# arcoslab/vfclik

Hardware: AMD Instinct MI355X
Metric: 7-DOF IK cycles/sec (whole node), batch=65536; max |qdot-qdot_ref| (higher is better)
Workload: dtype f64; 1 GPU; C3: batch=65536/GPU x 7-DOF lwr, goal + 8 decay repellers, float32 I/O, flags=0x0; parallelism=arm batch sharded over 1 GPU(s), no collective

## Files before the change

vfclik_amd/csrc/vfik_abi.cpp:

```cpp
#include <hip/hip_runtime.h>

#include <algorithm>
#include <cmath>
#include <cstdarg>
#include <cstdio>
#include <cstdlib>
#include <cstring>
#include <string>
#include <limits>
#include <vector>

#include "../../include/vfik.h"
#include "vfik_kernel.h"

namespace {

thread_local std::string g_err;

int fail(int code, const char* fmt, ...) {
    char buf[512];
    va_list ap;
    va_start(ap, fmt);
    vsnprintf(buf, sizeof buf, fmt, ap);
    va_end(ap);
// ... 381 lines not shown
    if (const char* e = std::getenv("VFIK_UNIFORM_IMAGE")) h->uni_allowed = std::atoi(e) != 0;
    if (const char* e = std::getenv("VFIK_MIXED_ORDERS")) h->mixed_allowed = std::atoi(e) != 0;
    if (const char* e = std::getenv("VFIK_DH_PATTERN")) h->dhp_allowed = std::atoi(e) != 0;
    if (const char* e = std::getenv("VFIK_ZERO_COPY_MAX")) h->zero_copy_max = (size_t)std::max(0L, std::atol(e));
    auto bail = [&](const char* what) { if (g_err.empty()) fail(VFIK_E_HIP, "%s failed", what); vfik_destroy(h); return (vfik_handle*)nullptr; };
    if (hipSetDevice(device) != hipSuccess) return bail("hipSetDevice");
    if (hipStreamCreateWithFlags(&h->stream, hipStreamNonBlocking) != hipSuccess) return bail("hipStreamCreate");
    {
        int cus = 0;
        if (hipDeviceGetAttribute(&cus, hipDeviceAttributeMultiprocessorCount, device) == hipSuccess && cus > 0) h->n_simd = 4 * cus;
    }
    const size_t B = batch;
    h->Bpad = (batch + 63) / 64 * 64;
    const size_t quad_plane = (size_t)h->Bpad * 4 * h->esz;
    {
        const size_t sz_goal = (4 + 6) * quad_plane;
        const size_t sz_kc = VFIK_KCONST_SLOT(vfik::kconst_bytes(n_joints));
        const size_t sz_lv = (size_t)((n_joints + 4) / 4) * h->Bpad * 4 * sizeof(float);
        const size_t sz_sf = (std::max<size_t>(1, (size_t)max_slots) + 1) / 2 * 3 * quad_plane;
        const size_t sz_su = (std::max<size_t>(1, (size_t)max_slots) + 1) * quad_plane;
        const size_t sz_sl = std::max<size_t>(1, (size_t)max_slots) * 2 * quad_plane;
        const size_t sz_or = (std::max<size_t>(1, (size_t)max_slots) + 15) / 16 * (size_t)h->Bpad * 16;
        if (dev_alloc(h, &h->d_arena, sz_goal + sz_kc + sz_lv + sz_sf + sz_su + sz_sl + sz_or, true)) return bail("alloc state arena");
        char* a0 = static_cast<char*>(h->d_arena);
        h->d_goal = a0;
        h->d_funnel = a0 + 4 * quad_plane;
        h->d_kconst = a0 + sz_goal;
        h->d_lastvec = reinterpret_cast<float*>(a0 + sz_goal + sz_kc);
        h->d_slots_fast = a0 + sz_goal + sz_kc + sz_lv;
        h->d_slots_uni = a0 + sz_goal + sz_kc + sz_lv + sz_sf;
        h->d_slots = a0 + sz_goal + sz_kc + sz_lv + sz_sf + sz_su;
        h->d_orders = a0 + sz_goal + sz_kc + sz_lv + sz_sf + sz_su + sz_sl;
    }
    {
        std::vector<char> plane((size_t)h->Bpad * 4 * h->esz, 0);
        for (int b = 0; b < h->Bpad; ++b) {
            if (io_dtype == 32) put<float>(plane, (size_t)b * 4 + 3, -std::numeric_limits<double>::infinity());
            else put<double>(plane, (size_t)b * 4 + 3, -std::numeric_limits<double>::infinity());
        }
        for (int sidx = 0; sidx < std::max(1, max_slots) + 1; ++sidx)
            if (hipMemcpyAsync(static_cast<char*>(h->d_slots_uni) + (size_t)sidx * plane.size(), plane.data(), plane.size(), hipMemcpyHostToDevice, h->stream) != hipSuccess)
                return bail("init uniform image");
        if (hipStreamSynchronize(h->stream) != hipSuccess) return bail("init uniform image");
    }
    if (dev_alloc(h, (void**)&h->d_mixw, 16 * sizeof(double), true)) return bail("alloc mixw");
    h->slots_per_arm.assign(B, 0);
    h->fast_slots_per_arm.assign(B, 0);
    h->arm_has_funnel.assign(B, 0);
    h->arm_pair_state.assign(B, 0);
    h->arm_safe.assign(B, 0.0);
    h->arm_force.assign(B, 0.0);
    h->arm_order.assign(B, -1);
#ifdef VFIK_STAMPS
    if (dev_alloc(h, (void**)&h->d_stamps, ((B + 63) / 64) * 10 * sizeof(unsigned long long), true)) return bail("alloc stamps");
#endif
    if (vfik_reset_state(h) != VFIK_OK) return bail("reset_state");
    vfik_params p{};
    p.speed_scale = 1.0; p.lambda = 0.1; p.rot_slowdown = 0.3; p.null_gain = 0.5; p.lookahead = 0.3;
    p.jl_gain = 0.5; p.max_vel = 1.0; p.jp_kp = 1.5; p.jp_delta = 0.087;
    for (double& w : p.wy) w = 1.0;
    for (double& w : p.wq) w = 1.0;
    p.mix_w[0] = p.mix_w[1] = 1.0;
    h->params = p;
    {
        std::vector<double> all(B, p.speed_scale);
        if (vfik_set_speed_scale(h, 0, batch, all.data()) != VFIK_OK) return bail("speed scale");
        h->speed_set = true;
    }
    if (hipStreamSynchronize(h->stream) != hipSuccess) return bail("sync");
    return h;
}

void vfik_destroy(vfik_handle* h) {
    if (!h) return;
    (void)hipSetDevice(h->device);
    if (h->stream) (void)hipStreamSynchronize(h->stream);
    void* ptrs[] = {h->d_arena, h->d_tool, h->d_ext, h->d_mixw, h->d_stamps, h->d_mixw_arm, h->d_track, h->d_wts, h->d_rollq[0], h->d_rollq[1], h->d_objects, h->d_obs_pose, h->d_obs_v6,
                    h->d_qalign};
    for (void* p : ptrs) if (p) (void)hipFree(p);
    if (h->arena_dev) (void)hipFree(h->arena_dev);
    if (h->arena_host) (void)hipHostFree(h->arena_host);
    for (auto& sc : h->sc) if (sc.p) (void)hipFree(sc.p);
    for (auto& ps : h->pipe) {
        if (ps.ev_out) (void)hipEventSynchronize(ps.ev_out);
        for (auto& s : ps.sc) if (s.p) (void)hipFree(s.p);
        for (hipEvent_t e : {ps.ev_in, ps.ev_k, ps.ev_out}) if (e) (void)hipEventDestroy(e);
    }
    if (h->s_in) (void)hipStreamDestroy(h->s_in);
    if (h->s_out) (void)hipStreamDestroy(h->s_out);
    if (h->own_stream && h->stream) (void)hipStreamDestroy(h->stream);
    delete h;
}

int vfik_set_stream(vfik_handle* h, void* hip_stream) {
    if (check_handle(h)) return VFIK_E_ARG;
    if (quiesce(h) != VFIK_OK) return VFIK_E_HIP;
    HIP_TRY(hipSetDevice(h->device));
    HIP_TRY(hipStreamSynchronize(h->stream));
    if (h->own_stream && h->stream) HIP_TRY(hipStreamDestroy(h->stream));
    h->stream = static_cast<hipStream_t>(hip_stream);
    h->own_stream = false;
    return VFIK_OK;
}

int vfik_set_chain(vfik_handle* h, const vfik_chain* c) {
    if (check_handle(h)) return VFIK_E_ARG;
    if (quiesce(h) != VFIK_OK) return VFIK_E_HIP;
// ... 782 lines not shown
}

int vfik_dev_free(vfik_handle* h, void* p) {
    if (check_handle(h)) return VFIK_E_ARG;
    HIP_TRY(hipSetDevice(h->device));
    HIP_TRY(hipFree(p));
    return VFIK_OK;
}

int vfik_memcpy_h2d(vfik_handle* h, void* dst, const void* src, size_t bytes) {
    if (check_handle(h)) return VFIK_E_ARG;
    HIP_TRY(hipSetDevice(h->device));
    HIP_TRY(hipMemcpyAsync(dst, src, bytes, hipMemcpyHostToDevice, h->stream));
    HIP_TRY(hipStreamSynchronize(h->stream));
    return VFIK_OK;
}

int vfik_memcpy_d2h(vfik_handle* h, void* dst, const void* src, size_t bytes) {
    if (check_handle(h)) return VFIK_E_ARG;
    HIP_TRY(hipSetDevice(h->device));
    HIP_TRY(hipMemcpyAsync(dst, src, bytes, hipMemcpyDeviceToHost, h->stream));
    HIP_TRY(hipStreamSynchronize(h->stream));
    return VFIK_OK;
}

int vfik_time_steps(vfik_handle* h, const vfik_io* io, int warmup, int steps, float* ms_total) {
    if (check_handle(h)) return VFIK_E_ARG;
    if (!ms_total || steps < 1 || warmup < 0) return fail(VFIK_E_ARG, "vfik_time_steps: bad arguments");
    HIP_TRY(hipSetDevice(h->device));
    for (int i = 0; i < warmup; ++i) {
        int rc = vfik_step(h, io);
        if (rc != VFIK_OK) return rc;
    }
    hipEvent_t t0, t1;
    HIP_TRY(hipEventCreate(&t0));
    HIP_TRY(hipEventCreate(&t1));
    HIP_TRY(hipEventRecord(t0, h->stream));
    for (int i = 0; i < steps; ++i) {
        int rc = vfik_step(h, io);
        if (rc != VFIK_OK) { (void)hipEventDestroy(t0); (void)hipEventDestroy(t1); return rc; }
    }
    HIP_TRY(hipEventRecord(t1, h->stream));
    HIP_TRY(hipEventSynchronize(t1));
    HIP_TRY(hipEventElapsedTime(ms_total, t0, t1));
    (void)hipEventDestroy(t0);
    (void)hipEventDestroy(t1);
    return VFIK_OK;
}

#ifdef VFIK_STAMPS
int vfik_debug_read_stamps(vfik_handle* h, unsigned long long* dst) {
    if (check_handle(h)) return VFIK_E_ARG;
    HIP_TRY(hipStreamSynchronize(h->stream));
    HIP_TRY(hipMemcpy(dst, h->d_stamps, (size_t)((h->B + 63) / 64) * 10 * sizeof(unsigned long long), hipMemcpyDeviceToHost));
    return VFIK_OK;
}
#endif

int vfik_slots_in_use(vfik_handle* h) { return h ? h->slots_used : VFIK_E_ARG; }

int vfik_field_path(vfik_handle* h) {
    if (!h) return VFIK_E_ARG;
    if (h->fast_order < 0) return 0;
    return h->any_funnel ? 2 : 1;
}

long vfik_launch_epoch(vfik_handle* h) { return h ? h->epoch : (long)VFIK_E_ARG; }

int vfik_dh_pattern(vfik_handle* h) { return h ? ((h->plain && !h->tool_per_arm && !h->d_wts) ? h->dhp : 0) : VFIK_E_ARG; }

int vfik_mixed_orders(vfik_handle* h) {
    if (!h) return VFIK_E_ARG;
    return (h->fast_order >= 0 && h->mixed) ? 1 : 0;
}

int vfik_uniform_repellers(vfik_handle* h) {
    if (!h) return VFIK_E_ARG;
    return (h->fast_order >= 0 && h->uni_ok && h->uni_allowed) ? 1 : 0;
}

int vfik_set_small_batch_kernel(vfik_handle* h, int max_batch) {
    if (check_handle(h)) return VFIK_E_ARG;
    if (max_batch < 0) return fail(VFIK_E_ARG, "max_batch must be >= 0");
    ++h->epoch;
    h->sub8_max_batch = max_batch;
    h->sub8_max_batch_full = max_batch;
    h->sub8_max_batch_ns = max_batch;
    return VFIK_OK;
}

long vfik_small_batch_launches(vfik_handle* h) { return h ? h->sub8_launches : -1; }

int vfik_launched_kernels(vfik_handle* h, char* buf, int len) {
    if (check_handle(h)) return VFIK_E_ARG;
    if (h->launched_lost) return fail(VFIK_E_STATE, "more than %d distinct cycle kernels launched since the last vfik_launched_kernels", vfik_handle::LAUNCHED_MAX);
    std::string all;
    for (int i = 0; i < h->launched_n; ++i) {
        all += vfik::cycle_kernel_name(h->launched[i].p, h->n, h->io_dtype, h->launched[i].ns);
        all += '\n';
    }
    if (!buf) return (int)all.size();
    if (len < (int)all.size() + 1) return fail(VFIK_E_ARG, "vfik_launched_kernels: %d bytes needed", (int)all.size() + 1);
    std::memcpy(buf, all.c_str(), all.size() + 1);
    h->launched_n = 0;
    return (int)all.size();
}

// ... 4 lines not shown
```

vfclik_amd/csrc/vfik_kernel.h:

```cpp
#pragma once
#include <algorithm>
#include <cstddef>
#include <cstdio>
#include <string>

#include <hip/hip_runtime.h>
#include <stdint.h>

#include "../../include/vfik_types.h"

#ifndef VFIK_NJ_LIST
#define VFIK_NJ_LIST X(6) X(7) X(10) X(14)
#endif

namespace vfik {

template <int NJ>
struct KConst {
    double base[12];
    struct DH { double off, crev, cprs, sprs, qd, d, a, ca, sa, pad; } dh[NJ];
    double tail_c, tail_s, tail_e;
    double rep_safe;
    double speed, lambda2, rot_slow, null_gain, lookahead, max_vel;
    double cos_slow;
// ... 7 lines not shown
    double q_hi[NJ];
    double q_mid[NJ];
    double inv_half[NJ];
    double jl_k[NJ];
    unsigned prismatic_mask;
    unsigned pad0;
    static constexpr int KIN_BYTES = (12 + 10 * NJ + 4 + 10 + VFIK_MIX_CHANNELS + 12 + 6 + NJ) * 8;
    static constexpr int KIN_ROWS = (KIN_BYTES + 1023) / 1024;
};
#define VFIK_KCONST_REP_FORCE_OFF ((12 + 9) * 8)
#define VFIK_KCONST_REP_SAFE_OFF(nj) ((12 + 10 * (nj) + 3) * 8)
static_assert(offsetof(KConst<7>, rep_safe) == VFIK_KCONST_REP_SAFE_OFF(7) && offsetof(KConst<14>, rep_safe) == VFIK_KCONST_REP_SAFE_OFF(14), "KConst::rep_safe");
static_assert(offsetof(KConst<7>, dh) + offsetof(KConst<7>::DH, pad) == VFIK_KCONST_REP_FORCE_OFF, "KConst::dh[0].pad");
static_assert(offsetof(KConst<7>, wq) + 7 * 8 == KConst<7>::KIN_BYTES && offsetof(KConst<14>, wq) + 14 * 8 == KConst<14>::KIN_BYTES, "KConst::wq closes the LDS-copied block");
static_assert(KConst<7>::KIN_BYTES <= 1024 && KConst<6>::KIN_BYTES <= 1024 && KConst<10>::KIN_BYTES <= 2048 && KConst<14>::KIN_BYTES <= 2048, "the copied block keeps its row count");
template <int NJ> struct KTab { static constexpr int OFFSET = ((int)sizeof(KConst<NJ>) + 1023) / 1024 * 1024; };

template <int NJ, int DHP> struct DhPattern { static constexpr unsigned SWAP = 0, NONE = 0, D0 = 0, OFF0 = 0, OFFPI = 0; static constexpr bool BASE_I = false; };
template <> struct DhPattern<7, 1> { static constexpr unsigned SWAP = 0x3Fu, NONE = 0x40u, D0 = 0x2Au, OFF0 = 0x15u, OFFPI = 0x6Au; static constexpr bool BASE_I = true; };
template <> struct DhPattern<14, 1> {
    static constexpr unsigned SWAP = 0x1FBFu, NONE = 0x2040u, D0 = 0x152Au, OFF0 = 0xA95u, OFFPI = 0x356Au;
    static constexpr bool BASE_I = true;
};
template <> struct DhPattern<6, 1> { static constexpr unsigned SWAP = 0x1Du, NONE = 0x20u, D0 = 0x16u, OFF0 = 0x27u, OFFPI = 0x18u; static constexpr bool BASE_I = true; };
int dh_pattern_of(int nj, unsigned swap, unsigned none, unsigned d0, unsigned off0, unsigned offpi, bool base_identity);

template <typename T> struct Stage {
    static constexpr int PRE = sizeof(T) == 8 ? 4 : 8;
    static constexpr int Q16 = (int)sizeof(T) / 4;
    static constexpr int QBYTES = 4 * (int)sizeof(T);
    static constexpr int QSTEP = Q16 * 1024;
    static constexpr int QPCF = 3 * PRE / 2;
    static constexpr int GOAL_OFF = 0, SLOT_OFF = 4 * QSTEP, Q_OFF = (4 + QPCF) * QSTEP;
    __host__ __device__ static constexpr int qbytes(int nj) { return nj * (int)sizeof(T); }
    __host__ __device__ static constexpr int q16(int nj) { return qbytes(nj) / 16; }
    __host__ __device__ static constexpr int qrem(int nj) { return qbytes(nj) % 16; }
    __host__ __device__ static constexpr int qregion(int nj) { return q16(nj) * 1024 + qrem(nj) * 64; }
    __host__ __device__ static constexpr int kin_rows(int nj) { return ((12 + 10 * nj + 4 + 10 + VFIK_MIX_CHANNELS + 12 + 6 + nj) * 8 + 1023) / 1024; }
    __host__ __device__ static constexpr int kin_off(int nj) { return Q_OFF + qregion(nj); }
    __host__ __device__ static constexpr int tab_off(int nj) { return kin_off(nj) + kin_rows(nj) * 1024; }
    __host__ __device__ static constexpr int lean_bytes(int nj) { return tab_off(nj) + 1024; }
    __host__ __device__ static constexpr int slot_off(int idx, int nj) {
        return idx < QPCF ? SLOT_OFF + idx * QSTEP : lean_bytes(nj) + (idx - QPCF) * QSTEP;
    }
    __host__ __device__ static constexpr int tool_off(int nj) { return lean_bytes(nj) + (2 * PRE - QPCF) * QSTEP; }
    __host__ __device__ static constexpr int mixw_off(int nj) { return tool_off(nj) + 3 * QSTEP; }
    __host__ __device__ static constexpr int bytes(int nj) { return mixw_off(nj) + 2 * QSTEP; }
};

#define VFIK_ROLL_MAX_NJ 7
#ifndef VFIK_HEAVY_MIN_NJ
#define VFIK_HEAVY_MIN_NJ 12
#endif

struct KArgs {
    int B;
    int Bpad;
    int slots_used;
    int fast_order;
    unsigned flags;
    int tool_stride;
    int plain;
    int block;
    const void* q;
    const void* goal;
    const void* slots;
    const void* slots_fast;
    const void* tool;
    const void* null_control;
    const void* ext;
    const void* mixw;
    const double* wts;
    const void* q_ref;
    const void* q_cmded;
    float* lastvec;
    void* qdot_vf;
    void* qdot_null;
    void* qdot_out;
    void* pose;
    void* pose_nt;
    void* v6;
    void* qdist;
    void* goal_dist;
    int* status;
    unsigned long long* stamps;
    const void* kc;
    void* q_out;
    double dt;
    int n_cycles;
    int clamp;
    int status_or;
    const int* active;
    const void* q_lo;
    const void* q_hi;
    void* q_ref_out;
    int sub8_max_batch;
    int sub8_max_batch_ns;
    int sub8_max_batch_full;
    int n_simd;
    const void* funnel;
    int slots_used_fast;
    int has_funnel;
    const void* arena;
    int uni;
    int uni_planes;
    int waves2;
// ... 233 lines not shown
```

vfclik_amd/csrc/vfik_kernel.hip:

```cpp
#include "vfik_kernel.h"

#include <algorithm>
#include <cmath>
#include <cstring>
#include <type_traits>

namespace vfik {
#define VFIK_CAT2(a, b) a##b
#define VFIK_CAT(a, b) VFIK_CAT2(a, b)
#if defined(VFIK_ONLY_NJ) && VFIK_ONLY_NJ >= VFIK_HEAVY_MIN_NJ
void VFIK_CAT(launch_heavy_nj, VFIK_ONLY_NJ)(int io_dtype, bool ns, const KArgs& a, const CyclePlan& p, hipStream_t stream);
#endif
namespace {

constexpr double EPS_LEN = 1e-12;
constexpr double D_FLOOR = 1e-9;
constexpr double MAG_CAP = 1e6;

__device__ __forceinline__ double rcp_nr(double x) {
    double y = __builtin_amdgcn_rcp(x);
    double e = __builtin_fma(-x, y, 1.0);
    y = __builtin_fma(y, e, y);
    e = __builtin_fma(-x, y, 1.0);
    return __builtin_fma(y, e, y);
// ... 487 lines not shown
        double z[NJ];
        descent(z);
        double c[6];
#pragma unroll
        for (int r = 0; r < 6; ++r) c[r] = 0.0;
#pragma unroll
        for (int i = 0; i < NJ; ++i)
#pragma unroll
            for (int r = 0; r < 6; ++r) c[r] += Jm[i][r] * z[i];
#pragma unroll
        for (int r = 0; r < 6; ++r)
#pragma unroll
            for (int i = 0; i < NJ; ++i) z[i] -= c[r] * Jm[i][r];
#pragma unroll
        for (int i = 0; i < NJ; ++i) qn[i] += z[i];
    }
    return advanced;
}


template <typename T, int NJ>
__device__ __forceinline__ int q_lds_off(int b, int lane) {
    constexpr int n16 = Stage<T>::q16(NJ), rem = Stage<T>::qrem(NJ);
    if (b < n16 * 16) return (b >> 4) * 1024 + lane * 16 + (b & 15);
    const int rb = b - n16 * 16;
    (void)rem;
    return n16 * 1024 + (rb >> 2) * 256 + lane * 4 + (rb & 3);
}

typedef __attribute__((address_space(1))) const void* GPtr;
typedef __attribute__((address_space(3))) void* LPtr;

template <typename T>
__device__ __forceinline__ void stage_quad(const char* gbase, unsigned voff, char* region, int off) {
    const char* gsrc = gbase + (long)(int)voff;
    __builtin_amdgcn_global_load_lds((GPtr)gsrc, (LPtr)(region + off), 16, 0, 2);
    if (Stage<T>::Q16 == 2) __builtin_amdgcn_global_load_lds((GPtr)(gsrc + 16), (LPtr)(region + off + 1024), 16, 0, 2);
}

template <typename T>
__device__ __forceinline__ void read_quad(const char* region, int off, int lane, double* out) {
    if (Stage<T>::Q16 == 1) {
        typedef float f4 __attribute__((ext_vector_type(4)));
        const f4 v = *reinterpret_cast<const f4*>(region + off + lane * 16);
        out[0] = (double)v.x; out[1] = (double)v.y; out[2] = (double)v.z; out[3] = (double)v.w;
    } else {
        typedef double d2 __attribute__((ext_vector_type(2)));
        const d2 lo = *reinterpret_cast<const d2*>(region + off + lane * 16);
        const d2 hi = *reinterpret_cast<const d2*>(region + off + 1024 + lane * 16);
        out[0] = lo.x; out[1] = lo.y; out[2] = hi.x; out[3] = hi.y;
    }
}

template <typename T> struct SlotGlobal {
    const T* sq; long Q;
    __device__ __forceinline__ double operator()(int m, int e) const { return slot_elem(sq, Q, m, e); }
};
template <typename T> struct SlotLds {
    const char* region; int lane; int nj;
    __device__ __forceinline__ double operator()(int m, int e) const {
        const int quad = 2 * m + (e >> 2), c = e & 3;
        const int off = Stage<T>::slot_off(quad, nj);
        if (Stage<T>::Q16 == 1)
            return (double)*reinterpret_cast<const float*>(region + off + lane * 16 + c * 4);
        return *reinterpret_cast<const double*>(region + off + (c >> 1) * 1024 + lane * 16 + (c & 1) * 8);
    }
};


#define HOTK(member) (NJ >= 10 ? klc->member : kc->member)

#define VFIK_WAIT_VM(N) asm volatile("s_waitcnt vmcnt(%0)" ::"n"(N) : "memory")

#ifdef VFIK_STAMPS
#define STAMP(i)                                                                                   \
    do {                                                                                           \
        __builtin_amdgcn_sched_barrier(0);                                                         \
        unsigned long long t_;                                                                     \
        asm volatile("s_memtime %0\n\ts_waitcnt lgkmcnt(0)" : "=s"(t_)::"memory");                   \
        __builtin_amdgcn_sched_barrier(0);                                                         \
        if ((threadIdx.x & 63) == 0) {                                                            \
            a.stamps[(long)(arm >> 6) * 10 + (i)] = t_;                                            \
            if ((i) == 0 || (i) == 7) a.stamps[(long)(arm >> 6) * 10 + 8 + ((i) != 0)] = __builtin_amdgcn_s_memrealtime(); \
        }                                                                                          \
    } while (0)
#define PIN(x) asm volatile("" : "+v"(x))
#define PIN_ARR(arr, n)                              \
    do {                                             \
        _Pragma("unroll") for (int i_ = 0; i_ < (n); ++i_) PIN((arr)[i_]); \
    } while (0)
#else
#define STAMP(i)
#define PIN(x)
#define PIN_ARR(arr, n)
#endif

#ifdef VFIK_STAMPS
template <int LEAN, bool ROLL, bool FASTF, bool MIXO = false> struct SmallArgs { static constexpr bool value = false; };
#else
template <int LEAN, bool ROLL, bool FASTF, bool MIXO = false> struct SmallArgs { static constexpr bool value = LEAN == 1 && !ROLL && FASTF && !MIXO; };
#endif
template <typename T, int NJ> struct ArenaLayout {
    __host__ __device__ static long funnel_off(long Bpad) { return 4 * Bpad * 4 * (long)sizeof(T); }
    __host__ __device__ static long kconst_off(long Bpad) { return (4 + 6) * Bpad * 4 * (long)sizeof(T); }
    __host__ __device__ static long lastvec_off(long Bpad) { return kconst_off(Bpad) + VFIK_KCONST_SLOT(KTab<NJ>::OFFSET + 1024); }
    __host__ __device__ static long slots_fast_off(long Bpad) { return lastvec_off(Bpad) + (long)((NJ + 4) / 4) * Bpad * 16; }
};

template <typename T, int NJ, bool NULLSP, bool PLAIN, bool ROLL, bool FASTF, int LEAN, int CF, bool PERS, bool FUN, int WAVES, bool UNI, bool MIXO, int DHP>
__device__ __forceinline__ void
cycle_body(const typename std::conditional<SmallArgs<LEAN, ROLL, FASTF, MIXO>::value, KLean, KArgs>::type& a_in) {
    static_assert(DHP == 0 || (PLAIN && FASTF && (!ROLL || LEAN == 1) && !PERS && LEAN != 0 && (sizeof(T) == 4 || DHP == 1)), "DHP: the lean straight-line variants (single cycle, a stepped rollout's cycle, and the lean rollout); the option bits: float32 I/O");
    static_assert(!(DHP & 2) || LEAN != 2, "TOOLC: not in a stepped rollout's cycle");
    static_assert(!(DHP & 2) || !ROLL, "TOOLC: single-cycle variants only (a rollout with a tool is stepped)");
    constexpr int DHPAT = DHP & 1;
    constexpr bool TOOLC = (DHP & 2) != 0;
    constexpr bool WTSC = (DHP & 4) != 0;
    static_assert(!WTSC || (NJ <= 7 && !ROLL && LEAN != 2), "WTSC: single-cycle variants of chains of up to 7 joints");
    constexpr bool WEIGHTED = !PLAIN || WTSC;
    static_assert(!MIXO || (FASTF && PLAIN && !ROLL && !PERS && !UNI && WAVES == 1 && (LEAN == 1 || LEAN == 3)), "MIXO: the lean single-cycle straight-line variants");
    static_assert(!PERS || (LEAN == 1 && FASTF && PLAIN && !ROLL && sizeof(T) == 4 && NJ <= 7 && !FUN), "PERS: lean straight-line float launches only");
    static_assert(!FUN || (FASTF && PLAIN && !ROLL && (LEAN == 1 || LEAN == 3)), "FUN: the lean single-cycle straight-line variants");
    static_assert(WAVES == 1 || (WAVES == 2 && LEAN == 1 && FASTF && PLAIN && !ROLL && !PERS && !FUN && sizeof(T) == 4 && NJ <= 7), "WAVES 2: lean straight-line float launches only");
    static_assert(!UNI || (FASTF && PLAIN && !ROLL && !PERS && !FUN && (LEAN == 1 || LEAN == 3)), "UNI: the lean single-cycle straight-line variants");
    KArgs a;
    if constexpr (SmallArgs<LEAN, ROLL, FASTF, MIXO>::value) {
        a = KArgs{};
        a.B = a_in.B; a.Bpad = a_in.Bpad; a.slots_used = a_in.slots_used; a.fast_order = a_in.fast_order; a.flags = a_in.flags; a.block = a_in.block;
        a.q = a_in.q; a.qdot_out = a_in.qdot_out; a.status = a_in.status;
        const char* const base = static_cast<const char*>(a_in.base);
        a.goal = base;
        a.funnel = base + ArenaLayout<T, NJ>::funnel_off(a_in.Bpad);
        a.kc = base + ArenaLayout<T, NJ>::kconst_off(a_in.Bpad);
        a.lastvec = reinterpret_cast<float*>(const_cast<char*>(base) + ArenaLayout<T, NJ>::lastvec_off(a_in.Bpad));
        a.slots_fast = base + ArenaLayout<T, NJ>::slots_fast_off(a_in.Bpad);
        a.slots = a.slots_fast;
    } else {
        a = a_in;
    }
    if constexpr (UNI) {
        a.slots_fast = static_cast<const char*>(a.slots_fast) + (long)(a.fast_order >> 8) * a.Bpad * (4 * (long)sizeof(T));
        a.fast_order &= 255;
    }
    if constexpr (CF >= 0) a.flags = (unsigned)CF;
    if constexpr (LEAN != 0) {
// ... 378 lines not shown
                }
            }
            if (PLAIN) {
                Jm[i][0] = cx; Jm[i][1] = cy; Jm[i][2] = cz;
            } else {
                const bool pris = (kc->prismatic_mask >> i) & 1u;
                Jm[i][0] = pris ? Jm[i][3] : cx; Jm[i][1] = pris ? Jm[i][4] : cy; Jm[i][2] = pris ? Jm[i][5] : cz;
                Jm[i][3] = pris ? 0.0 : Jm[i][3]; Jm[i][4] = pris ? 0.0 : Jm[i][4]; Jm[i][5] = pris ? 0.0 : Jm[i][5];
            }
        }
    }

    PIN_ARR(R, 9); PIN_ARR(p, 3);
#pragma unroll
    for (int i = 0; i < NJ; ++i) { PIN_ARR(Jm[i], 6); }
    STAMP(3);
    double Rt[9], pt[3], rr[3];
    if (PLAIN) {
#pragma unroll
        for (int k = 0; k < 9; ++k) Rt[k] = R[k];
#pragma unroll
        for (int k = 0; k < 3; ++k) { pt[k] = p[k]; rr[k] = 0.0; }
        if constexpr (TOOLC) {
            double tl[12];
#pragma unroll
            for (int k = 0; k < 12; ++k) tl[k] = HOTK(tool[k]);
#pragma unroll
            for (int r = 0; r < 3; ++r) {
                const double x = Rt[3 * r], y = Rt[3 * r + 1], z = Rt[3 * r + 2];
#pragma unroll
                for (int c = 0; c < 3; ++c) Rt[3 * r + c] = x * tl[c] + y * tl[4 + c] + z * tl[8 + c];
                pt[r] += x * tl[3] + y * tl[7] + z * tl[11];
            }
        }
    } else {
        double tl[12];
        if (a.tool_stride) {
#pragma unroll
            for (int k = 0; k < 3; ++k) read_quad<T>(region, Stage<T>::tool_off(NJ) + k * Stage<T>::QSTEP, lanec, tl + 4 * k);
        } else {
#pragma unroll
            for (int k = 0; k < 12; ++k) tl[k] = kc->tool[k];
        }
#pragma unroll
        for (int r = 0; r < 3; ++r) {
#pragma unroll
            for (int c = 0; c < 3; ++c) Rt[3 * r + c] = R[3 * r] * tl[c] + R[3 * r + 1] * tl[4 + c] + R[3 * r + 2] * tl[8 + c];
            rr[r] = -(R[3 * r] * tl[3] + R[3 * r + 1] * tl[7] + R[3 * r + 2] * tl[11]);
            pt[r] = p[r] - rr[r];
        }
    }

    constexpr bool EARLY_FACTOR = NJ <= 7;
    const double* wts = (!PLAIN && a.wts) ? a.wts + arm : nullptr;
    const long wpitch = a.Bpad;
    double A[6][6], dinv[6];
    double G[FUSEP ? 6 : 1][6], wn[6];
    double wyv[WEIGHTED ? 6 : 1];
    auto wq2_of = [&](int i) {
        const double wqi = wts ? wts[(long)(6 + i) * wpitch] : kc->wq[i];
        return wqi * wqi;
    };
    auto ik_factor = [&]() {
        if constexpr (WEIGHTED) {
#pragma unroll
            for (int r = 0; r < 6; ++r) wyv[WEIGHTED ? r : 0] = wts ? wts[(long)r * wpitch] : kc->wy[r];
        }
        constexpr bool GFROMA = FUSEP && PLAIN && !GLATE;
        if constexpr (ACCJ) {
#pragma unroll
            for (int r = 0; r < 6; ++r) {
                if constexpr (!GLATE) wn[r] = wne[r];
#pragma unroll
                for (int c = 0; c <= r; ++c) A[r][c] = Ae[ACCJ ? r : 0][c];
                if constexpr (!GFROMA) A[r][r] += HOTK(lambda2);
            }
        } else {
#pragma unroll
            for (int r = 0; r < 6; ++r)
#pragma unroll
                for (int c = 0; c <= r; ++c) A[r][c] = (r == c && !GFROMA && !WEIGHTED) ? HOTK(lambda2) : 0.0;
            if constexpr (FUSEP && !GLATE) {
#pragma unroll
                for (int r = 0; r < 6; ++r) {
                    wn[r] = 0.0;
#pragma unroll
                    for (int c = 0; c <= r; ++c) G[r][c] = 0.0;
                }
            }
#pragma unroll
            for (int i = 0; i < NJ; ++i) {
                double t[6];
                if constexpr (WEIGHTED) {
                    const double w2 = wq2_of(i);
#pragma unroll
                    for (int r = 0; r < 6; ++r) t[r] = w2 * Jm[i][r];
                }
#pragma unroll
                for (int r = 0; r < 6; ++r) {
                    if (jzero(i, r)) continue;
#pragma unroll
                    for (int c = 0; c <= r; ++c)
                        if (!jzero(i, c)) A[r][c] = __builtin_fma(WEIGHTED ? t[r] : Jm[i][r], Jm[i][c], A[r][c]);
                    if constexpr (FUSEP && !GLATE) {
                        wn[r] = __builtin_fma(Jm[i][r], zp[i], wn[r]);
                        if constexpr (!PLAIN) {
#pragma unroll
                            for (int c = 0; c <= r; ++c) G[FUSEP ? r : 0][c] = __builtin_fma(Jm[i][r], Jm[i][c], G[FUSEP ? r : 0][c]);
                        }
                    }
                }
            }
            if constexpr (WEIGHTED) {
#pragma unroll
                for (int r = 0; r < 6; ++r)
#pragma unroll
                    for (int c = 0; c <= r; ++c) A[r][c] = __builtin_fma(wyv[WEIGHTED ? r : 0] * wyv[WEIGHTED ? c : 0], A[r][c], r == c ? HOTK(lambda2) : 0.0);
            }
        }
        if constexpr (GFROMA) {
#pragma unroll
            for (int r = 0; r < 6; ++r) {
#pragma unroll
                for (int c = 0; c <= r; ++c) G[FUSEP ? r : 0][c] = A[r][c];
                A[r][r] += HOTK(lambda2);
            }
        }
#pragma unroll
        for (int j = 0; j < 6; ++j) {
            double v[6];
#pragma unroll
            for (int k = 0; k < j; ++k) v[k] = A[j][k] * A[k][k];
            double dj = A[j][j];
#pragma unroll
            for (int k = 0; k < j; ++k) dj = __builtin_fma(-A[j][k], v[k], dj);
            A[j][j] = dj;
            dinv[j] = rcp_1nr(dj);
#pragma unroll
            for (int k = 0; k < j; ++k)
#pragma unroll
                for (int i = j + 1; i < 6; ++i) A[i][j] = __builtin_fma(-A[i][k], v[k], A[i][j]);
#pragma unroll
            for (int i = j + 1; i < 6; ++i) A[i][j] *= dinv[j];
        }
    };
    if constexpr (EARLY_FACTOR) ik_factor();

    double tot[6] = {0, 0, 0, 0, 0, 0}, sc[2] = {1.0, 1.0};
    double gdist[2] = {0.0, 0.0};
    double speed;
    if (PERS && has_next) VFIK_WAIT_VM(N_SLOT + NPF);
    else
    VFIK_WAIT_VM(N_SLOT);
    {
        double gq[16];
#pragma unroll
        for (int k = 0; k < 4; ++k) read_quad<T>(dreg, Stage<T>::GOAL_OFF + k * Stage<T>::QSTEP, lanec, gq + 4 * k);
        speed = gq[15];
        {
            double GR[9], Gp[3];
#pragma unroll
            for (int r = 0; r < 3; ++r) {
#pragma unroll
                for (int c = 0; c < 3; ++c) GR[3 * r + c] = gq[4 * r + c];
                Gp[r] = gq[4 * r + 3];
            }
            attractor(Rt, pt, GR, Gp, gq[13], gq[14], HOTK(rot_slow), a.goal_dist ? -2.0 : HOTK(cos_slow), gq[12] != 0.0, tot, sc, gdist);
        }
    }
    if constexpr (FUN) {
        double f[12];
#pragma unroll
        for (int k = 0; k < 3; ++k) read_quad<T>(region, FUN_OFF + k * Stage<T>::QSTEP, lanec, f + 4 * k);
        double an, ainv;
        sqrt_rsqrt(f[3] * f[3] + f[4] * f[4] + f[5] * f[5], an, ainv);
        const bool on = f[11] != 0.0 && an > EPS_LEN;
        const double ax = f[3] * ainv, ay = f[4] * ainv, az = f[5] * ainv;
        const double wx = pt[0] - f[0], wy = pt[1] - f[1], wz = pt[2] - f[2];
        const double along = wx * ax + wy * ay + wz * az;
        const double ex = wx - along * ax, ey = wy - along * ay, ez = wz - along * az;
        double P, Pinv, dist, dinv;
        sqrt_rsqrt(ex * ex + ey * ey + ez * ez, P, Pinv);
        sqrt_rsqrt(wx * wx + wy * wy + wz * wz, dist, dinv);
        Pinv = P < D_FLOOR ? 1.0 / D_FLOOR : Pinv;
        dinv = dist < D_FLOOR ? 1.0 / D_FLOOR : dinv;
        const double phi = atan2_pos(P, on ? along : 1.0);
        const double cutA = f[6];
        const double ga = cutA > 0.0 ? fmin(1.0, pow_order(phi * rcp_nr(cutA > 0.0 ? cutA : 1.0), on ? f[7] : 1.0)) : 1.0;
        const double gd = fmin(1.0, pow_order(f[8] * dinv, on ? f[9] : 1.0));
        const double kf = on ? -f[10] * ga * gd * Pinv : 0.0;
        tot[0] += on ? ex * kf : 0.0; tot[1] += on ? ey * kf : 0.0; tot[2] += on ? ez * kf : 0.0;
        double g[12];
#pragma unroll
        for (int k = 0; k < 3; ++k) read_quad<T>(region, FUN_OFF + (3 + k) * Stage<T>::QSTEP, lanec, g + 4 * k);
        if (__any(g[9] != 0.0)) {
            double nn, ninv;
            sqrt_rsqrt(g[3] * g[3] + g[4] * g[4] + g[5] * g[5], nn, ninv);
            const bool hon = g[9] != 0.0 && nn > EPS_LEN;
            const double hh = ((pt[0] - g[0]) * g[3] + (pt[1] - g[1]) * g[4] + (pt[2] - g[2]) * g[5]) * ninv;
            const double hmag = fmin(pow_order(g[6] * rcp_nr(fmax(hon ? hh : 1.0, D_FLOOR)), hon ? g[7] : 1.0), MAG_CAP);
            const double kh = hon ? -g[8] * hmag * ninv : 0.0;
            tot[0] += hon ? g[3] * kh : 0.0; tot[1] += hon ? g[4] * kh : 0.0; tot[2] += hon ? g[5] * kh : 0.0;
        }
    }
    PIN_ARR(tot, 6); PIN_ARR(sc, 2);
    STAMP(4);
    {
        const T* sq = static_cast<const T*>(a.slots) + (long)arm * 4;
        const long Qp = Bp * 4;
        if constexpr (FASTF) {
            const int n0 = a.fast_order;
            auto chunk = [&](int c0) {
                const int ncur = a.slots_used - c0;
                double dx[PRE], dy[PRE], dz[PRE], rs[PRE], fk[PRE];
                unsigned ow[MIXO ? PRE / 4 : 1];
                if constexpr (MIXO) {
                    const char* orow = region + ORD_OFF + lanec * 16 + (c0 & 15);
#pragma unroll
                    for (int u = 0; u < PRE / 4; ++u) ow[u] = *reinterpret_cast<const unsigned*>(orow + 4 * u);
                }
                if constexpr (UNI) {
                    const double usafe = kl->rep_safe, uforce = kl->dh[0].pad;
#pragma unroll
                    for (int m = 0; m < PRE; ++m) {
                        double v[4];
                        read_quad<T>(dreg, Stage<T>::slot_off(m, NJ), lanec, v);
                        dx[m] = v[0] - pt[0];
                        dy[m] = v[1] - pt[1];
                        dz[m] = v[2] - pt[2];
                        rs[m] = fmax(v[3] + usafe, 0.0);
                        fk[m] = uforce;
                    }
                } else
#pragma unroll
                for (int k = 0; k < PRE / 2; ++k) {
                    double v[12];
#pragma unroll
                    for (int u = 0; u < 3; ++u) read_quad<T>(dreg, Stage<T>::slot_off(3 * k + u, NJ), lanec, v + 4 * u);
#pragma unroll
                    for (int hf = 0; hf < 2; ++hf) {
                        const int m = 2 * k + hf;
                        dx[m] = v[6 * hf] - pt[0];
                        dy[m] = v[6 * hf + 1] - pt[1];
                        dz[m] = v[6 * hf + 2] - pt[2];
                        rs[m] = v[6 * hf + 3] + v[6 * hf + 4];
                        fk[m] = m < ncur ? v[6 * hf + 5] : 0.0;
                    }
                }
                if (c0 + PRE < a.slots_used) {
                    asm volatile("s_waitcnt lgkmcnt(0)" ::: "memory");
#pragma unroll
                    for (int idx = 0; idx < QPC; ++idx) {
                        const int m = UNI ? c0 + PRE + idx : c0 + PRE + 2 * (idx / 3);
                        const char* sm = slots0 + (m < a.slots_used ? (long)(UNI ? c0 + PRE + idx + 1 : (c0 + PRE) / 2 * 3 + idx) * planeB : 0);
                        stage_quad<T>(sm, (unsigned)arm * (unsigned)QB, dreg, Stage<T>::slot_off(idx, NJ));
                    }
                    if constexpr (MIXO) issue_orders(c0 + PRE);
                }
                double di[PRE], rb[PRE], rp[PRE];
#pragma unroll
                for (int m = 0; m < PRE; ++m) {
                    di[m] = fmin(rsqrt_1nr_pos(__builtin_fma(dx[m], dx[m], __builtin_fma(dy[m], dy[m], __builtin_fma(dz[m], dz[m], 1e-300)))), 1.0 / D_FLOOR);
                    rb[m] = rs[m] * di[m];
                    rp[m] = 1.0;
                }
                if constexpr (MIXO) {
                    unsigned su[PRE / 4];
                    bool agree = true;
#pragma unroll
                    for (int u = 0; u < PRE / 4; ++u) {
                        su[u] = (unsigned)__builtin_amdgcn_readfirstlane((int)ow[MIXO ? u : 0]);
                        agree = agree && __all(ow[MIXO ? u : 0] == su[u]);
                    }
                    bool lanes = !agree;
                    if (agree) {
                        bool all5 = true;
#pragma unroll
                        for (int u = 0; u < PRE / 4; ++u) all5 = all5 && su[u] == 0x05050505u;
                        auto order_of = [&](int m) { return ((m < 4 ? su[0] : su[PRE / 4 - 1]) >> (8 * (m & 3))) & 127u; };
                        auto fifth = [&](double* dst) {
#pragma unroll
                            for (int m = 0; m < PRE; ++m) { const double b2 = rb[m] * rb[m]; dst[m] = b2 * b2 * rb[m]; }
                        };
                        const unsigned o1 = order_of(0);
                        unsigned todo = 0, rest = 0, o2 = o1;
                        if (!all5) {
#pragma unroll
                            for (int m = 1; m < PRE; ++m) todo |= (order_of(m) != o1 ? 1u : 0u) << m;
                            if (todo) {
                                o2 = order_of(__builtin_ctz(todo));
#pragma unroll
                                for (int m = 1; m < PRE; ++m) rest |= ((todo >> m) & 1u && order_of(m) != o2 ? 1u : 0u) << m;
                            }
                        }
                        lanes = rest != 0;
                        if (all5) {
                            fifth(rp);
                        } else if (!lanes) {
                            auto raise_all = [&](unsigned o, double* dst) {
                                if (o <= 1) {
#pragma unroll
                                    for (int m = 0; m < PRE; ++m) dst[m] = o ? rb[m] : 1.0;
                                    return;
                                }
                                int k = 30 - __builtin_clz(o);
#pragma unroll
                                for (int m = 0; m < PRE; ++m) dst[m] = rb[m] * rb[m];
                                for (;;) {
                                    if ((o >> k) & 1u) {
#pragma unroll
                                        for (int m = 0; m < PRE; ++m) dst[m] *= rb[m];
// ... 13 lines not shown
                                    for (int m = 0; m < PRE; ++m) pw[m] = rp[m] * rp[m];
                                    for (unsigned r = ratio >> 1; r > 1; r >>= 1) {
#pragma unroll
                                        for (int m = 0; m < PRE; ++m) pw[m] *= pw[m];
                                    }
                                } else {
                                    raise_all(o2, pw);
                                }
#pragma unroll
                                for (int m = 1; m < PRE; ++m) rp[m] = (todo >> m) & 1u ? pw[m] : rp[m];
                            }
                        }
                    }
                    if (lanes) {
                        int nn[PRE], nmax = 0;
#pragma unroll
                        for (int m = 0; m < PRE; ++m) { nn[m] = (int)((ow[MIXO ? (m >> 2) : 0] >> (8 * (m & 3))) & 127u); nmax |= nn[m]; }
                        int top = 0;
#pragma unroll
                        for (int k = 0; k < 7; ++k)
                            if (__any((nmax >> k) != 0)) top = k + 1;
                        for (int k = 0; k < top; ++k) {
#pragma unroll
                            for (int m = 0; m < PRE; ++m) rp[m] = (nn[m] >> k) & 1 ? rp[m] * rb[m] : rp[m];
                            if (k + 1 < top) {
#pragma unroll
                                for (int m = 0; m < PRE; ++m) rb[m] *= rb[m];
                            }
                        }
                    }
                } else
                if (n0 == 5) {
#pragma unroll
                    for (int m = 0; m < PRE; ++m) { const double b2 = rb[m] * rb[m]; rp[m] = b2 * b2 * rb[m]; }
                } else {
                for (int e = n0; e;) {
                    if (e & 1) {
#pragma unroll
                        for (int m = 0; m < PRE; ++m) rp[m] *= rb[m];
                    }
                    e >>= 1;
                    if (e) {
#pragma unroll
                        for (int m = 0; m < PRE; ++m) rb[m] *= rb[m];
                    }
                }
                }
#pragma unroll
                for (int m = 0; m < PRE; ++m) {
                    const double k = fk[m] * fmin(rp[m], MAG_CAP) * di[m];
                    tot[0] += dx[m] * k; tot[1] += dy[m] * k; tot[2] += dz[m] * k;
                }
            };
            if (PERS && has_next) VFIK_WAIT_VM(NPF);
            else VFIK_WAIT_VM(0);
            chunk(0);
            for (int c0 = PRE; c0 < a.slots_used; c0 += PRE) {
                VFIK_WAIT_VM(0);
                chunk(c0);
            }
        } else {
            const SlotLds<T> rl{dreg, lanec, NJ};
            const double rs = HOTK(rot_slow), csl = HOTK(cos_slow);
            for (int c0 = 0; c0 < a.slots_used; c0 += PRE) {
                if (c0 > 0) {
                    asm volatile("s_waitcnt lgkmcnt(0)" ::: "memory");
#pragma unroll
                    for (int idx = 0; idx < 2 * PRE; ++idx) {
                        const int m = c0 + (idx >> 1);
                        const char* sm = slots0 + (m < a.slots_used ? (long)m * 2 * planeB : 0) + (idx & 1) * planeB;
                        stage_quad<T>(sm, (unsigned)arm * (unsigned)QB, dreg, Stage<T>::slot_off(idx, NJ));
                    }
                }
                VFIK_WAIT_VM(0);
                const int ncur = a.slots_used - c0 < PRE ? a.slots_used - c0 : PRE;
                const SlotGlobal<T> rg{sq + (long)c0 * 2 * Qp, Qp};
                unsigned done = 0;
                {
                    double dx[PRE], dy[PRE], dz[PRE], rsum[PRE], fk[PRE], di[PRE], rb[PRE], rp[PRE];
                    int nn[PRE];
                    int nmax = 0;
#pragma unroll
                    for (int m = 0; m < PRE; ++m) {
                        double s0[4], s1[4];
                        read_quad<T>(dreg, Stage<T>::slot_off(2 * m, NJ), lanec, s0);
                        read_quad<T>(dreg, Stage<T>::slot_off(2 * m + 1, NJ), lanec, s1);
                        const int n = (int)s1[1];
                        const bool ok = m < ncur && (int)s1[3] == VFIK_FIELD_REPELLER && (double)n == s1[1] && n >= 0 && n < 128;
                        dx[m] = s0[0] - pt[0]; dy[m] = s0[1] - pt[1]; dz[m] = s0[2] - pt[2];
                        rsum[m] = s0[3] + s1[0];
                        fk[m] = ok ? s1[2] : 0.0;
                        nn[m] = ok ? n : 0;
                        nmax |= nn[m];
                        done |= ok ? (1u << m) : 0u;
                    }
#pragma unroll
                    for (int m = 0; m < PRE; ++m) {
                        di[m] = fmin(rsqrt_1nr(dx[m] * dx[m] + dy[m] * dy[m] + dz[m] * dz[m]), 1.0 / D_FLOOR);
                        rb[m] = rsum[m] * di[m];
                        rp[m] = 1.0;
                    }
                    int top = 0;
#pragma unroll
                    for (int k = 0; k < 7; ++k)
                        if (__any((nmax >> k) != 0)) top = k + 1;
                    for (int k = 0; k < top; ++k) {
#pragma unroll
                        for (int m = 0; m < PRE; ++m) rp[m] = (nn[m] >> k) & 1 ? rp[m] * rb[m] : rp[m];
                        if (k + 1 < top) {
#pragma unroll
                            for (int m = 0; m < PRE; ++m) rb[m] *= rb[m];
                        }
// ... 1421 lines not shown
```

Before: 15.38 billion cycles/s.

## Interleave normal-equation and LDL factorisation into memory-wait gaps of the goal and slot loads

Splits the IK normal-matrix accumulation and the LDL factorisation into ranged pieces. On the plain fast-field path it schedules these pieces between the global-memory wait, the LDS goal reads and the first repeller chunk, so the arithmetic hides load latency instead of running up front. Raw LDS reads are separated from their conversion, and scheduling barriers plus register holds keep the ordering in place. This raises register pressure and depends on the compiler honouring the barriers. It also adds optional per-wait timing stamps, which are compiled out by default.

```diff
diff --git a/vfclik_amd/csrc/vfik_abi.cpp b/vfclik_amd/csrc/vfik_abi.cpp
--- a/vfclik_amd/csrc/vfik_abi.cpp
+++ b/vfclik_amd/csrc/vfik_abi.cpp
@@ -457,7 +457,7 @@
     h->arm_force.assign(B, 0.0);
     h->arm_order.assign(B, -1);
 #ifdef VFIK_STAMPS
-    if (dev_alloc(h, (void**)&h->d_stamps, ((B + 63) / 64) * 10 * sizeof(unsigned long long), true)) return bail("alloc stamps");
+    if (dev_alloc(h, (void**)&h->d_stamps, ((B + 63) / 64) * VFIK_STAMP_STRIDE * sizeof(unsigned long long), true)) return bail("alloc stamps");
 #endif
     if (vfik_reset_state(h) != VFIK_OK) return bail("reset_state");
     vfik_params p{};
@@ -1346,7 +1346,7 @@
 int vfik_debug_read_stamps(vfik_handle* h, unsigned long long* dst) {
     if (check_handle(h)) return VFIK_E_ARG;
     HIP_TRY(hipStreamSynchronize(h->stream));
-    HIP_TRY(hipMemcpy(dst, h->d_stamps, (size_t)((h->B + 63) / 64) * 10 * sizeof(unsigned long long), hipMemcpyDeviceToHost));
+    HIP_TRY(hipMemcpy(dst, h->d_stamps, (size_t)((h->B + 63) / 64) * VFIK_STAMP_STRIDE * sizeof(unsigned long long), hipMemcpyDeviceToHost));
     return VFIK_OK;
 }
 #endif
diff --git a/vfclik_amd/csrc/vfik_kernel.h b/vfclik_amd/csrc/vfik_kernel.h
--- a/vfclik_amd/csrc/vfik_kernel.h
+++ b/vfclik_amd/csrc/vfik_kernel.h
@@ -83,6 +83,7 @@
 #ifndef VFIK_HEAVY_MIN_NJ
 #define VFIK_HEAVY_MIN_NJ 12
 #endif
+#define VFIK_STAMP_STRIDE 20
 
 struct KArgs {
     int B;
diff --git a/vfclik_amd/csrc/vfik_kernel.hip b/vfclik_amd/csrc/vfik_kernel.hip
--- a/vfclik_amd/csrc/vfik_kernel.hip
+++ b/vfclik_amd/csrc/vfik_kernel.hip
@@ -563,6 +563,29 @@
     }
 }
 
+template <typename T> struct RawQuad;
+template <> struct RawQuad<float> { typedef float f4 __attribute__((ext_vector_type(4))); f4 v; };
+template <> struct RawQuad<double> { typedef double d2 __attribute__((ext_vector_type(2))); d2 lo, hi; };
+template <typename T>
+__device__ __forceinline__ RawQuad<T> load_quad(const char* region, int off, int lane) {
+    RawQuad<T> r;
+    if constexpr (Stage<T>::Q16 == 1) {
+        r.v = *reinterpret_cast<const typename RawQuad<T>::f4*>(region + off + lane * 16);
+    } else {
+        r.lo = *reinterpret_cast<const typename RawQuad<T>::d2*>(region + off + lane * 16);
+        r.hi = *reinterpret_cast<const typename RawQuad<T>::d2*>(region + off + 1024 + lane * 16);
+    }
+    return r;
+}
+template <typename T>
+__device__ __forceinline__ void cvt_quad(const RawQuad<T>& r, double* out) {
+    if constexpr (Stage<T>::Q16 == 1) {
+        out[0] = (double)r.v.x; out[1] = (double)r.v.y; out[2] = (double)r.v.z; out[3] = (double)r.v.w;
+    } else {
+        out[0] = r.lo.x; out[1] = r.lo.y; out[2] = r.hi.x; out[3] = r.hi.y;
+    }
+}
+
 template <typename T> struct SlotGlobal {
     const T* sq; long Q;
     __device__ __forceinline__ double operator()(int m, int e) const { return slot_elem(sq, Q, m, e); }
@@ -583,6 +606,9 @@
 
 #define VFIK_WAIT_VM(N) asm volatile("s_waitcnt vmcnt(%0)" ::"n"(N) : "memory")
 
+template <int N> using IC = std::integral_constant<int, N>;
+#define VFIK_HOLD(x) asm volatile("" : "+v"(x))
+
 #ifdef VFIK_STAMPS
 #define STAMP(i)                                                                                   \
     do {                                                                                           \
@@ -591,9 +617,26 @@
         asm volatile("s_memtime %0\n\ts_waitcnt lgkmcnt(0)" : "=s"(t_)::"memory");                   \
         __builtin_amdgcn_sched_barrier(0);                                                         \
         if ((threadIdx.x & 63) == 0) {                                                            \
-            a.stamps[(long)(arm >> 6) * 10 + (i)] = t_;                                            \
-            if ((i) == 0 || (i) == 7) a.stamps[(long)(arm >> 6) * 10 + 8 + ((i) != 0)] = __builtin_amdgcn_s_memrealtime(); \
+            a.stamps[(long)(arm >> 6) * VFIK_STAMP_STRIDE + (i)] = t_;                                            \
+            if ((i) == 0 || (i) == 7) a.stamps[(long)(arm >> 6) * VFIK_STAMP_STRIDE + 8 + ((i) != 0)] = __builtin_amdgcn_s_memrealtime(); \
         }                                                                                          \
+    } while (0)
+#define WSTAMP_STORE(k, t0_, t1_)                                                                  \
+    if ((threadIdx.x & 63) == 0) {                                                                 \
+        a.stamps[(long)(arm >> 6) * VFIK_STAMP_STRIDE + 10 + 2 * (k)] = t0_;                       \
+        a.stamps[(long)(arm >> 6) * VFIK_STAMP_STRIDE + 11 + 2 * (k)] = t1_;                       \
+    }
+#define WSTAMP_VM(k, N)                                                                            \
+    do {                                                                                           \
+        unsigned long long t0_, t1_;                                                               \
+        asm volatile("s_memtime %0\n\ts_waitcnt vmcnt(%2)\n\ts_memtime %1\n\ts_waitcnt lgkmcnt(0)" : "=&s"(t0_), "=&s"(t1_) : "n"(N) : "memory"); \
+        WSTAMP_STORE(k, t0_, t1_)                                                                  \
+    } while (0)
+#define WSTAMP_LGKM(k)                                                                             \
+    do {                                                                                           \
+        unsigned long long t0_, t1_;                                                               \
+        asm volatile("s_memtime %0\n\ts_waitcnt lgkmcnt(0)\n\ts_memtime %1\n\ts_waitcnt lgkmcnt(0)" : "=&s"(t0_), "=&s"(t1_)::"memory"); \
+        WSTAMP_STORE(k, t0_, t1_)                                                                  \
     } while (0)
 #define PIN(x) asm volatile("" : "+v"(x))
 #define PIN_ARR(arr, n)                              \
@@ -602,6 +645,8 @@
     } while (0)
 #else
 #define STAMP(i)
+#define WSTAMP_VM(k, N) VFIK_WAIT_VM(N)
+#define WSTAMP_LGKM(k)
 #define PIN(x)
 #define PIN_ARR(arr, n)
 #endif
@@ -1086,6 +1131,8 @@
     }
 
     constexpr bool EARLY_FACTOR = NJ <= 7;
+    constexpr bool FILL = EARLY_FACTOR && !ACCJ && PLAIN && FASTF && !ROLL && !PERS && WAVES == 1 && (LEAN == 1 || LEAN == 3);
+    constexpr int FILL_NI = 3, FILL_J = 3;
     const double* wts = (!PLAIN && a.wts) ? a.wts + arm : nullptr;
     const long wpitch = a.Bpad;
     double A[6][6], dinv[6];
@@ -1095,13 +1142,17 @@
         const double wqi = wts ? wts[(long)(6 + i) * wpitch] : kc->wq[i];
         return wqi * wqi;
     };
-    auto ik_factor = [&]() {
+    auto ik_normal = [&](auto i0c, auto i1c) {
+        constexpr int I0 = decltype(i0c)::value, I1 = decltype(i1c)::value;
+        constexpr bool GFROMA = FUSEP && PLAIN && !GLATE;
+        if constexpr (I0 == 0) {
         if constexpr (WEIGHTED) {
 #pragma unroll
             for (int r = 0; r < 6; ++r) wyv[WEIGHTED ? r : 0] = wts ? wts[(long)r * wpitch] : kc->wy[r];
         }
-        constexpr bool GFROMA = FUSEP && PLAIN && !GLATE;
+        }
         if constexpr (ACCJ) {
+            static_assert(!ACCJ || (I0 == 0 && I1 == NJ), "ACCJ: A is complete when the factorisation starts");
 #pragma unroll
             for (int r = 0; r < 6; ++r) {
                 if constexpr (!GLATE) wn[r] = wne[r];
@@ -1110,6 +1161,7 @@
                 if constexpr (!GFROMA) A[r][r] += HOTK(lambda2);
             }
         } else {
+            if constexpr (I0 == 0) {
 #pragma unroll
             for (int r = 0; r < 6; ++r)
 #pragma unroll
@@ -1122,8 +1174,9 @@
                     for (int c = 0; c <= r; ++c) G[r][c] = 0.0;
                 }
             }
-#pragma unroll
-            for (int i = 0; i < NJ; ++i) {
+            }
+#pragma unroll
+            for (int i = I0; i < I1; ++i) {
                 double t[6];
                 if constexpr (WEIGHTED) {
                     const double w2 = wq2_of(i);
@@ -1145,14 +1198,14 @@
                     }
                 }
             }
-            if constexpr (WEIGHTED) {
+            if constexpr (WEIGHTED && I1 == NJ) {
 #pragma unroll
                 for (int r = 0; r < 6; ++r)
 #pragma unroll
                     for (int c = 0; c <= r; ++c) A[r][c] = __builtin_fma(wyv[WEIGHTED ? r : 0] * wyv[WEIGHTED ? c : 0], A[r][c], r == c ? HOTK(lambda2) : 0.0);
             }
         }
-        if constexpr (GFROMA) {
+        if constexpr (GFROMA && I1 == NJ) {
 #pragma unroll
             for (int r = 0; r < 6; ++r) {
 #pragma unroll
@@ -1160,8 +1213,10 @@
                 A[r][r] += HOTK(lambda2);
             }
         }
-#pragma unroll
-        for (int j = 0; j < 6; ++j) {
+    };
+    auto ik_ldl = [&](auto j0c, auto j1c) {
+#pragma unroll
+        for (int j = decltype(j0c)::value; j < decltype(j1c)::value; ++j) {
             double v[6];
 #pragma unroll
             for (int k = 0; k < j; ++k) v[k] = A[j][k] * A[k][k];
@@ -1178,18 +1233,47 @@
             for (int i = j + 1; i < 6; ++i) A[i][j] *= dinv[j];
         }
     };
-    if constexpr (EARLY_FACTOR) ik_factor();
+    auto ik_factor = [&]() {
+        ik_normal(IC<0>{}, IC<NJ>{});
+        ik_ldl(IC<0>{}, IC<6>{});
+    };
+    if constexpr (EARLY_FACTOR && !FILL) ik_factor();
 
     double tot[6] = {0, 0, 0, 0, 0, 0}, sc[2] = {1.0, 1.0};
     double gdist[2] = {0.0, 0.0};
     double speed;
+    auto hold_A = [&]() {
+#pragma unroll
+        for (int r = 0; r < 6; ++r)
+#pragma unroll
+            for (int c = 0; c <= r; ++c) VFIK_HOLD(A[r][c]);
+    };
+    (void)hold_A;
+    if constexpr (FILL) {
+        ik_normal(IC<0>{}, IC<NJ - FILL_NI>{});
+        hold_A();
+    }
     if (PERS && has_next) VFIK_WAIT_VM(N_SLOT + NPF);
     else
-    VFIK_WAIT_VM(N_SLOT);
+    WSTAMP_VM(0, N_SLOT);
     {
         double gq[16];
-#pragma unroll
-        for (int k = 0; k < 4; ++k) read_quad<T>(dreg, Stage<T>::GOAL_OFF + k * Stage<T>::QSTEP, lanec, gq + 4 * k);
+        if constexpr (FILL) {
+            RawQuad<T> graw[4];
+#pragma unroll
+            for (int k = 0; k < 4; ++k) graw[k] = load_quad<T>(dreg, Stage<T>::GOAL_OFF + k * Stage<T>::QSTEP, lanec);
+            __builtin_amdgcn_sched_barrier(0);
+            ik_normal(IC<NJ - FILL_NI>{}, IC<NJ>{});
+            hold_A();
+            __builtin_amdgcn_sched_barrier(0);
+            WSTAMP_LGKM(1);
+#pragma unroll
+            for (int k = 0; k < 4; ++k) cvt_quad<T>(graw[k], gq + 4 * k);
+        } else {
+#pragma unroll
+            for (int k = 0; k < 4; ++k) read_quad<T>(dreg, Stage<T>::GOAL_OFF + k * Stage<T>::QSTEP, lanec, gq + 4 * k);
+            WSTAMP_LGKM(1);
+        }
         speed = gq[15];
         {
             double GR[9], Gp[3];
@@ -1244,7 +1328,7 @@
         const long Qp = Bp * 4;
         if constexpr (FASTF) {
             const int n0 = a.fast_order;
-            auto chunk = [&](int c0) {
+            auto chunk = [&](int c0, auto first_c) {
                 const int ncur = a.slots_used - c0;
                 double dx[PRE], dy[PRE], dz[PRE], rs[PRE], fk[PRE];
                 unsigned ow[MIXO ? PRE / 4 : 1];
@@ -1291,6 +1375,14 @@
                     }
                     if constexpr (MIXO) issue_orders(c0 + PRE);
                 }
+                if constexpr (FILL && decltype(first_c)::value) {
+                    ik_ldl(IC<FILL_J>{}, IC<6>{});
+                    hold_A();
+#pragma unroll
+                    for (int j = 0; j < 6; ++j) VFIK_HOLD(dinv[j]);
+                    __builtin_amdgcn_sched_barrier(0);
+                }
+                if constexpr (decltype(first_c)::value) WSTAMP_LGKM(3);
                 double di[PRE], rb[PRE], rp[PRE];
 #pragma unroll
                 for (int m = 0; m < PRE; ++m) {
@@ -1410,12 +1502,16 @@
                     tot[0] += dx[m] * k; tot[1] += dy[m] * k; tot[2] += dz[m] * k;
                 }
             };
+            if constexpr (FILL) {
+                ik_ldl(IC<0>{}, IC<FILL_J>{});
+                hold_A();
+            }
             if (PERS && has_next) VFIK_WAIT_VM(NPF);
-            else VFIK_WAIT_VM(0);
-            chunk(0);
+            else WSTAMP_VM(2, 0);
+            chunk(0, IC<1>{});
             for (int c0 = PRE; c0 < a.slots_used; c0 += PRE) {
                 VFIK_WAIT_VM(0);
-                chunk(c0);
+                chunk(c0, IC<0>{});
             }
         } else {
             const SlotLds<T> rl{dreg, lanec, NJ};
```

Measured after the change: 15.40 billion cycles/s, median of 2. About the same (+0.2%).
